# cvxgrp/cvxpygen

Measured on AMD Instinct MI355X. Metric: QP instances solved/sec (batched MPC QP, OSQP; inputs resident in HBM), higher is better.
Workload: dtype f64

## Files before the change

### cvxpygen_amd/codegen.py

```python

from __future__ import annotations

import os
import shutil
import subprocess
from typing import List, Optional, Sequence

import numpy as np

from .solve_program import GEN_EXTRA_SLOTS, LANES, RaggedProgram, execution_steps, padded_offsets_fit

CSRC = os.path.join(os.path.dirname(os.path.abspath(__file__)), 'csrc')


class ProgramTooLarge(Exception):
    """the family's solve program cannot be made LDS-resident: no specialised library for it"""


def emit_program_header(rp: RaggedProgram, name: str = 'family', plan=None, depth: int = 2, cross: int = 4,
                        pad_offsets: bool = False, group_offsets: int = 4, batch: int = 1, early: int = 4) -> str:
    out: List[str] = []
    w = out.append
    w(f'// Generated by cvxpygen_amd.codegen for problem family "{name}" -- do not edit.')
    w(f'// solve program: {rp.n_phases} phases, {rp.n_chunks} chunks, {int(rp.ctab[:, 0].sum())} steps, '
# ... 504 lines not shown
                    if int(rp.ctab[c, 3]) & 2:
                        w(f'        const double o{c} = w[r{c} & CPG_GEN_SLOT_MASK];')
                w('        cpgw::sched_fence();')
                nsteps_c = {}
                for _, c in lst:
                    nsteps_c[c] = nsteps_c.get(c, 0) + 1
                kacc = {c: (1 if (n_ < 6 or not TEAM_SPLIT_SUMS) else (2 if n_ < 12 else 4)) for c, n_ in nsteps_c.items()}
                seen, first = {}, {}
                for t, c in lst:
                    cx = f'cf[{reg_of[t]}]' if coef == 'reg' else f'c{t}'
                    j = seen.get(c, 0) % kacc[c]
                    seen[c] = seen.get(c, 0) + 1
                    nm = f'a{c}' if kacc[c] == 1 else f'a{c}_{j}'
                    if (c, j) not in first:
                        first[(c, j)] = True
                        w(f'        double {nm} = {cx} * x{t};' if coef == 'reg' else f'        double {nm} = fma({cx}, x{t}, 0.0);')
                    else:
                        w(f'        {nm} = fma({cx}, x{t}, {nm});')
                for c in chunks:
                    if kacc[c] == 2:
                        w(f'        const double a{c} = a{c}_0 + a{c}_1;')
                    elif kacc[c] == 4:
                        w(f'        const double a{c} = (a{c}_0 + a{c}_1) + (a{c}_2 + a{c}_3);')
                for c in chunks:
                    lg, kind = int(rp.ctab[c, 1]), int(rp.ctab[c, 3])
                    assert not kind & 4, 'a team executor has no deferred phases (resident_plan: intra phases instead)'
                    red = f'cpgw::seg_sum_first_lit<{lg}>(a{c}, {_mask_literals(stage_masks(rp, c, shift_of[c]))})' if kind & 1 else f'cpgw::group_sum_first<{lg}>(a{c})'
                    acc = f'o{c} + ' if kind & 2 else ''
                    w(f'        w[r{c} & CPG_GEN_SLOT_MASK] = {acc}{red};')
            if sync:
                w('        cpgw::block_sync();')
        w('    } break;')
    w('    default: {')
    if sync:
        for _ in plist:
            w('        cpgw::block_sync();')
    w('    } break;')
    w('    }')
    w('}')
    w('}  // namespace cpg')
    return '\n'.join(out) + '\n' + epilogue


def factor_fingerprint(fac) -> int:
    h = 0x811C9DC5
    ct = np.asarray(fac.ctab, dtype=np.int32).reshape(-1, 4)[:, [0, 1, 3]]
    for arr in (np.ascontiguousarray(ct), np.ascontiguousarray(fac.tlen, dtype=np.uint32)):
        for b in arr.tobytes():
            h = ((h ^ b) * 0x01000193) & 0xFFFFFFFF
    return h


FACTOR_LOOKAHEAD = int(os.environ.get('CPG_FACTOR_LOOKAHEAD', 3))


def emit_factor_program(fac, nnzL: int, N: int, prefix: str = 'GENI', lookahead: Optional[int] = None,
                        preloaded: bool = False, func: str = 'numeric_ldl_gen', zero: Optional[int] = None, body: bool = True,
                        one: Optional[int] = None, inverse_from: Optional[int] = None) -> str:
    G = f'CPG_{prefix}_FAC'
    P = FACTOR_LOOKAHEAD if lookahead is None else lookahead
    ct = np.asarray(fac.ctab, dtype=np.int64).reshape(-1, 4)
    nch = ct.shape[0]
    first = np.concatenate([[0], np.cumsum(ct[:, 0])])
    out = []
    w = out.append
    w(f'#define {G}_NCHUNKS {nch}')
    w(f'#define {G}_NSTEPS {int(first[-1])}')
    w(f'#define {G}_FINGERPRINT {factor_fingerprint(fac)}u')
    w(f'#define {G}_ZERO {nnzL + N if zero is None else int(zero)}')
    if one is not None:
        w(f'#define {G}_ONE {int(one)}')
    inv0 = nch if inverse_from is None else int(inverse_from)
    w(f'#define {G}_CHUNKS {{' + ', '.join(f'{{{int(L)}, {int(last)}, {int(lg)}}}' for L, last, _, lg in ct) + '}')
    if not body:
        return '\n'.join(out) + '\n'
    w(f'#define {G}_GENERATED 1')
    w('namespace cpg {')
    if preloaded:
        w(f'CPG_DEV void {func}(const unsigned long long *tri, const unsigned *dk, double *w, int lane) {{')
    else:
        w(f'CPG_DEV void {func}(const unsigned long long *tri, const unsigned *dk, const double *kct, const double *rinv,')
        w('                             double *w, int lane) {')
    w('    const unsigned ln = (unsigned)cpgw::opaque(lane);     // (table addresses computed here, not hoisted out of the instance loop)')

    def req_dk(c):
        if c < nch:
            w(f'    const unsigned d{c} = cpgw::gld(dk, {c * 64}u + ln);')

    def req_rest(c):
        if c < nch:
            if not preloaded and c < inv0:
                w(f'    const double kc{c} = cpgw::gld(kct, {c * 64}u + ln);')
                w(f'    const double kr{c} = cpgw::gld(rinv, (d{c} >> 16) ? (d{c} >> 16) - 1u : 0u);')
            for s_ in range(int(ct[c, 0])):
                w(f'    const unsigned long long e{int(first[c]) + s_} = cpgw::gld(tri, {(int(first[c]) + s_) * 64}u + ln);')
    for c in range(2 * P):
        req_dk(c)
    for c in range(P):
        req_rest(c)
    for c in range(nch):
        L, last, _, lg = (int(v) for v in ct[c])
        last &= 1
        w(f'    // chunk {c}: {L} step(s), groups of {1 << lg}' + (', level end' if last else ''))
        req_dk(c + 2 * P)
        req_rest(c + P)
        if preloaded and L == 0:
            if last:
                w('    cpgw::lds_order();')
            continue
        w(f'    double a{c} = 0.0;')
        for s_ in range(L):
            e = f'e{int(first[c]) + s_}'
            w(f'    a{c} = fma(w[(unsigned){e} & 0xFFFFu] * w[(unsigned)({e} >> 32)], w[((unsigned){e} >> 16)], a{c});')
        w(f'    a{c} = cpgw::group_sum_first<{lg}>(a{c});')
        w(f'    if ((d{c} & 0xFFFFu) != 0xFFFFu) {{')
        if c >= inv0 and not preloaded:
            w(f'        w[d{c} & 0xFFFFu] = -a{c};')
        elif preloaded:
            w(f'        const double v = w[d{c} & 0xFFFFu] - a{c};')
            w(f'        w[d{c} & 0xFFFFu] = (d{c} >> 16) ? 1.0 / v : v;')
        else:
            w(f'        const double v = (kc{c} - ((d{c} >> 16) ? kr{c} : 0.0)) - a{c};')
            w(f'        w[d{c} & 0xFFFFu] = (d{c} & 0xFFFFu) >= {nnzL}u ? 1.0 / v : v;')
        w('    }')
        if last:
            w('    cpgw::lds_order();')
    w('    cpgw::lds_order();')
    w('}')
# ... 89 lines not shown
    else:
        sh = stream_header(plan, out_dir, name)
        if sh is not None:
            defs.append(f'-DCPG_GENS_HEADER="{sh}"')
    return hdr, defs


GENS_MAX_STEPS = int(os.environ.get('CPG_GENS_MAX_STEPS', 1200))
GENS_LOOKAHEAD = int(os.environ.get('CPG_GENS_LOOKAHEAD', 16))


def stream_header(plan, out_dir: str, name: str = 'family') -> Optional[str]:
    from . import refactor_plan as _rp
    from .solve_program import execution_steps
    d = plan.desc
    if not matrix_parameters(d) or os.environ.get('CPG_GENS', '0') != '1':
        return None
    rpl = _rp.build_refactor_plan(d.P, d.A, plan.osqp)
    T = len(execution_steps(rpl.sol))
    if T == 0 or T > GENS_MAX_STEPS or any(int(k_) & ~1 for k_ in rpl.sol.ctab[:, 3]):
        return None
    text = emit_instance_program(rpl.sol, name, lookahead=GENS_LOOKAHEAD, prefix='GENS', func='run_program_gens', coef='mem')
    path = os.path.join(os.path.abspath(out_dir), f'cpg_stream_{name}.h')
    if not (os.path.exists(path) and open(path).read() == text):
        with open(path, 'w') as f:
            f.write(text)
    return path


GENI_MAX_REGS = int(os.environ.get('CPG_GENI_MAX_REGS', 64))
GENI_MAX_STEPS = int(os.environ.get('CPG_GENI_MAX_STEPS', 240))
LDS_BYTES = 160 * 1024


SHARED_REG_LDS_REGS = 20


def shared_register_lds_bytes(n: int, m: int, n_steps: int, n_chunks: int, n_slots: int, n_regs: int, waves: int = 8) -> int:
    tab = 2 * (256 * ((n_steps + 3) // 4) + 256 * ((n_chunks + 3) // 4))
    return 8 * (n + m) + tab + 8 * 64 * min(SHARED_REG_LDS_REGS, n_regs) + waves * 8 * (n_slots + GEN_EXTRA_SLOTS)


def instance_program_fits(rpl) -> bool:
    mg = getattr(rpl, 'merged', None)
    rp = mg.sol if mg is not None else rpl.sol
    N = rpl.n + rpl.m
    steps = execution_steps(rp)
    if len(steps) > GENI_MAX_STEPS or rp.n_slots + GEN_EXTRA_SLOTS > 0x1FFF or not np.array_equal(rp.final_pos, np.arange(N)):
        return False
    if pack_step_registers(rp, steps)[2] > GENI_MAX_REGS:
        return False
    tab = 2 * (256 * ((len(steps) + 3) // 4) + 256 * ((rp.n_chunks + 3) // 4))
    per_wave = rp.n_slots + GEN_EXTRA_SLOTS + N + (N & 1)
    fac = rpl.nnzL + N
    if mg is not None:
        fac = mg.fac_len
        if fac >= 0xFFFF:
            return False
    per_wave = max(per_wave, fac + (fac & 1))
    return tab + 8 * 8 * per_wave <= LDS_BYTES


def instance_header(plan, out_dir: str, name: str = 'family') -> Optional[str]:
    from . import refactor_plan as _rp
    d = plan.desc
    o = plan.osqp_shared or plan.osqp
    Ps, As = o.pruned(d.P, d.A)
    rpl = _rp.shared_mode_plan(Ps, As, o)
    if not instance_program_fits(rpl):
        return None
    dims = dict(N=d.n_var, M=d.m, NEQ=d.n_eq)
    mg = rpl.merged
    if mg is None:
        prog, fac = rpl.sol, emit_factor_program(rpl.fac, rpl.nnzL, rpl.n + rpl.m)
    else:
        import types
        dims['NNZX'] = mg.nnzX
        prog = mg.sol
        fac = emit_factor_program(types.SimpleNamespace(ctab=mg.f_ctab, tlen=mg.f_len), rpl.nnzL, rpl.n + rpl.m,
                                  zero=mg.fac_len - 1, one=mg.one_pos, inverse_from=mg.base.fac.n_chunks)
    return write_instance_header(prog, os.path.join(os.path.abspath(out_dir), f'cpg_instance_{name}.h'), name,
                                 row_programs=shared_row_programs(Ps, As), dims=dims, epilogue=fac, lean=True)


RESIDENT_MAX_REGS = int(os.environ.get('CPG_RESIDENT_MAX_REGS', 160))
RESIDENT_MAX_STEPS = int(os.environ.get('CPG_RESIDENT_MAX_STEPS', 320))
RESIDENT_ACC_BASE = int(os.environ.get('CPG_RESIDENT_ACC_BASE', 32))
RESIDENT_GATHER_BATCH = int(os.environ.get('CPG_RESIDENT_GATHER_BATCH', 12))
RESIDENT_ACC_PAIRS = int(os.environ.get('CPG_RESIDENT_ACC_PAIRS', 112))


def resident_compiler_flags(defs: Sequence[str]) -> List[str]:
    return []


def matrix_parameters(desc) -> bool:
    import scipy.sparse as _sps
    NP = desc.NP
    return any(_sps.csr_matrix(desc.maps[k])[:, :NP].nnz > 0 for k in ('P', 'A'))


def resident_program_fits(rpl, np_var: Optional[int] = None) -> bool:
    rp = rpl.sol
    b = rpl.base
    N = b.n + b.m
    steps = execution_steps(rp)
    if len(steps) > RESIDENT_MAX_STEPS or not np.array_equal(rp.final_pos, np.arange(N)):
        return False
    if pack_step_registers(rp, steps)[2] > RESIDENT_MAX_REGS:
        return False
    tab = 2 * (256 * ((len(steps) + 3) // 4) + 256 * ((rp.n_chunks + 3) // 4))
    np_var = b.nnzP + b.nnzA + N if np_var is None else np_var
    slice_ = max(rpl.fac_len, rpl.w_slots + N, b.nnzA + b.nnzP + max(np_var, N + max(b.n, b.m)))
    slice_ += slice_ & 1
    return 8 * slice_ <= 0xFFFF and tab + 2 * 8 * slice_ <= LDS_BYTES


def resident_four_waves(rpl, np_var: int) -> bool:
    if os.environ.get('CPG_RES_FOUR_WAVES', '0') != '1':
        return False
    b = rpl.base
    N = b.n + b.m
    slice_ = max(rpl.fac_len, rpl.w_slots + b.m, max(b.nnzA + b.nnzP, max(np_var, N + max(b.n, b.m))))
    slice_ += slice_ & 1
    return 4 * 8 * slice_ <= LDS_BYTES


def resident_header(plan, out_dir: str, name: str = 'family') -> Optional[str]:
    from . import resident_plan as _rs
    d = plan.desc
    if not matrix_parameters(d):
        return None
    rpl = _rs.build_resident_plan(d.P, d.A, plan.osqp)
# ... 686 lines not shown
```

### cvxpygen_amd/csrc/cpg_hip.cpp

```cpp
#include "../../include/cpg_hip.h"

#include <math.h>
#include <stdio.h>
#include <stdlib.h>
#include <string.h>

#include <algorithm>
#include <string>
#include <type_traits>
#include <vector>

#include "cpg_osqp_kernel.h"
#include "cpg_osqp_refactor.h"
#include "cpg_osqp_resident.h"
#include "cpg_osqp_team.h"
#include "cpg_osqp_squad.h"
#include "cpg_clarabel_kernel.h"

#include <hip/hip_runtime.h>
typedef hipStream_t rt_stream_t;
typedef hipEvent_t rt_event_t;
#define RT_CHECK(expr)                                                                         \
    do {                                                                                       \
        hipError_t e_ = (expr);                                                                \
// ... 431 lines not shown
static int launch_squad(cpg_handle_t h, const cpg::DevBatch &Bt, int blocks, size_t lds) {
    const int nsx = (h->F.n + 63) / 64, nsz = (h->F.m + 63) / 64, nv = vary_slots(h);
#define Y(a, b, v, g, wm)                                                                         \
    if (nsx == a && nsz == b && (nv <= v || (v >= a && v >= b)) && g == 1)                        \
        return launch_kernel(osqp_squad_kernel<a, b, v>, blocks, CPG_GENQ_W * 64, lds, h->stream, h->F, h->U, h->S, Bt);
    CPG_KERNELS_LDS(Y)
#undef Y
    set_error("no compiled squad kernel for this family size");
    return CPG_E_UNSUPPORTED;
}
#endif

#if defined(CPG_GENI_HEADER) && defined(CPG_GENI_NNZX)
static int shared_reg_waves(cpg_handle_t h) { return h->waves_per_block > 0 && h->waves_per_block < 8 ? h->waves_per_block : 8; }
static size_t shared_reg_lds(cpg_handle_t h, int W) {
    const size_t tab = (size_t)(((CPG_GENI_NSTEPS + 3) / 4) * 256 + ((CPG_GENI_NCHUNKS + 3) / 4) * 256) * sizeof(unsigned short);
    return (size_t)(h->F.n + h->F.m) * sizeof(double) + tab + (size_t)cpg::SharedRegExec::nlds * 64 * sizeof(double) +
           (size_t)W * (CPG_GENI_NSLOTS + CPG_GEN_EXTRA_SLOTS) * sizeof(double);
}
static bool shared_reg_usable(cpg_handle_t h) {
    return !h->refactor_mode && !h->conic && h->sreg_ok && h->sreg_rho == h->F.rho && h->sreg_sigma == h->F.sigma &&
           h->inst_per_wave == 1 && shared_reg_lds(h, shared_reg_waves(h)) <= h->lds_limit;
}
static int launch_shared_reg(cpg_handle_t h, const cpg::DevBatch &Bt, int blocks, int waves, size_t lds) {
    const int nsx = (h->F.n + 63) / 64, nsz = (h->F.m + 63) / 64, nv = vary_slots(h);
#define Y(a, b, v, g, wm)                                                                         \
    if (nsx <= a && nsz <= b && (nv <= v || (v >= a && v >= b)) && g == 1)                        \
        return launch_kernel(osqp_shared_reg_kernel<a, b, v>, blocks, waves * 64, lds, h->stream, h->F, h->U, h->S, Bt, h->SRg);
    CPG_KERNELS_LDS(Y)
#undef Y
    set_error("no compiled register-executor kernel for this family size");
    return CPG_E_UNSUPPORTED;
}
#else
static bool shared_reg_usable(cpg_handle_t) { return false; }
#endif

static cpg::DevBatch make_batch(int64_t B, const double *d_theta, const double *d_state_in, double *d_state_out, double *d_prim,
                                double *d_dual, double *d_obj, int32_t *d_iter, int32_t *d_status, double *d_pri, double *d_dua) {
    cpg::DevBatch Bt;
    Bt.scratch = nullptr; Bt.state_in = d_state_in; Bt.state_out = d_state_out;
    Bt.B = B; Bt.theta = d_theta; Bt.prim = d_prim; Bt.dual = d_dual; Bt.obj = d_obj; Bt.pri_res = d_pri;
    Bt.dua_res = d_dua; Bt.iter = d_iter; Bt.status = d_status; Bt.counter = nullptr;
    Bt.ho_list = nullptr; Bt.ho_count = nullptr; Bt.ho_state = nullptr; Bt.list = nullptr; Bt.list_count = nullptr; Bt.resume = 0;
    return Bt;
}

#ifdef CPG_GENI_HEADER
static size_t instance_kernel_lds(const cpg_solver_s *h) {
    const size_t tab = (size_t)(((CPG_GENI_NSTEPS + 3) / 4) * 256 + ((CPG_GENI_NCHUNKS + 3) / 4) * 256) * sizeof(unsigned short);
    const size_t nq = (size_t)(h->F.n + h->F.m);
    size_t per_wave = (size_t)(CPG_GENI_NSLOTS + CPG_GEN_EXTRA_SLOTS) + nq + (nq & 1);
#ifdef CPG_GENI_FAC_NSTEPS
    const size_t fac = (size_t)CPG_GENI_FAC_ZERO + 1;
#else
    const size_t fac = (size_t)h->R.nnzL + nq;
#endif
    if (per_wave < fac) per_wave = fac + (fac & 1);
    return tab + 8 * per_wave * sizeof(double);
}
static bool instance_kernel_fits(const cpg_solver_s *h) {
    return h->R.gi_ok && h->program_in_lds != 0 && h->program_in_lds != 2 && instance_kernel_lds(h) <= h->lds_limit;
}
#endif

static int launch_per_instance(cpg_handle_t h, rt_stream_t stream, const cpg::DevSettings &S, cpg::DevBatch &Bt) {
    int rc;
    auto scratch = [&](int blocks, int waves, size_t doubles) {
        const int r = ensure(h->scratch, (size_t)blocks * waves * doubles * sizeof(double));
        Bt.scratch = (double *)h->scratch.p;
        return r;
    };
#ifdef CPG_GENT_HEADER
    if (h->Rs.ok == 2 && !h->R.shared_mats && h->program_in_lds != 0 && h->program_in_lds != 2) {
        const size_t lds = ((size_t)CPG_TEAM_SLICE_OFF + (size_t)h->Rs.slice_doubles) * sizeof(double);
        if (lds <= h->lds_limit) {
            long long per_cu = (long long)(h->lds_limit / lds);
            if (per_cu * CPG_GENT_W > 16) per_cu = 16 / CPG_GENT_W;
            if (CPG_GENT_W <= 4 && per_cu * CPG_GENT_W > 4) per_cu = 4 / CPG_GENT_W;
            if (h->blocks_per_cu > 0 && per_cu > h->blocks_per_cu) per_cu = h->blocks_per_cu;
            const int blocks = std::max(1, grid_blocks(h, Bt.B, 1, per_cu));
            if ((rc = scratch(blocks, 1, h->Rs.buf_doubles))) return rc;
            return launch_kernel(osqp_team_kernel, blocks, CPG_GENT_W * 64, lds, stream, h->F, h->R, h->Rs, S, Bt);
        }
    }
#endif
#ifdef CPG_GENR_HEADER
    if (h->Rs.ok && !h->R.shared_mats && h->program_in_lds != 0 && h->program_in_lds != 2) {
#ifdef CPG_GENR_TABLES_GLOBAL
        const size_t tab = 0;
#else
        const size_t tab = (size_t)(((CPG_GENR_NSTEPS + 3) / 4) * 256 + ((CPG_GENR_NCHUNKS + 3) / 4) * 256) * sizeof(unsigned short);
#endif
        const size_t slice = (size_t)h->Rs.slice_doubles * sizeof(double);
        int NW = h->waves_per_block > 0 ? h->waves_per_block : 4;
        if (NW > 4) NW = 4;
        while (NW > 1 && tab + (size_t)NW * slice > h->lds_limit) NW--;
        const size_t lds = tab + (size_t)NW * slice;
        if (lds <= h->lds_limit) {
            const int blocks = grid_blocks(h, Bt.B, NW, 1);
            if ((rc = scratch(blocks, NW, h->Rs.buf_doubles))) return rc;
            if (slot_class(h, rc, [&](auto NSX, auto NSZ) {
                    return launch_kernel(osqp_resident_kernel<NSX, NSZ>, blocks, NW * 64, lds, stream, h->F, h->R, h->Rs, S, Bt); }))
                return rc;
        }
    }
#endif
// ... 981 lines not shown
#ifdef CPG_GENI_NNZX
    const bool merged_lib = true;
#else
    const bool merged_lib = false;
#endif
    if (!(geni_dims && (g.nnzX > 0) == merged_lib && g.sol_chunks == CPG_GENI_NCHUNKS && g.sol_nnz == CPG_GENI_NNZ && g.sol_slots == CPG_GENI_NSLOTS))
        return CPG_OK;
    const size_t nd = (size_t)r->nnzL + N, nx = (size_t)g.nnzX;
    const unsigned hsh = program_fingerprint(g.sol_ctab, g.sol_desc, g.sol_cols, g.sol_chunks, g.sol_nnz);
    static const int steps[][4] = CPG_GENI_STEPS;
    static const int chunk_shift[] = CPG_GENI_CHUNK_SHIFT;
    bool ok = hsh == CPG_GENI_FINGERPRINT;
    {
        const int nn[3] = {CPG_GENI_AROWS_N, CPG_GENI_PROWS_N, CPG_GENI_ATROWS_N};
        for (int k = 0; ok && k < 3; k++) {
            if ((int)h->rows_hdr[k].size() != 4 * nn[k]) ok = false;
            for (int c2 = 0; ok && c2 < nn[k]; c2++)
                if (h->rows_hdr[k][4 * c2] != cpg::GeniRows::len(k, c2) || h->rows_hdr[k][4 * c2 + 3] != cpg::GeniRows::off(k, c2)) ok = false;
        }
    }
    if (ok) ok = generated_tables(g.sol_ctab, g.sol_desc, g.sol_cols, g.sol_chunks, g.sol_nnz, g.sol_slots, steps, CPG_GENI_NSTEPS, gcols, grows, chunk_shift, geni_row_bytes);
    if (ok) {
        gsrc.assign((size_t)CPG_GENI_NREGS * 64, 0u);
        glcol.assign((size_t)CPG_GENI_NREGS * 64, (unsigned short)0);
        std::vector<char> taken((size_t)CPG_GENI_NREGS * 64, 0);
        for (int t = 0; ok && t < CPG_GENI_NSTEPS; t++) {
            const int e = steps[t][0], cnt = steps[t][1], reg = steps[t][2], sh = steps[t][3];
            if (reg < 0 || reg >= CPG_GENI_NREGS) { ok = false; break; }
            for (int l = 0; l < cnt; l++) {
                int kind = g.sol_kind[e + l], idx = g.sol_idx[e + l];
                if (kind == 4) {
                    if (idx < 0 || (size_t)idx >= nx) { ok = false; break; }
                    kind = 3; idx += (int)N;
                }
                if (kind < 0 || kind > 3 || idx < 0 || idx >= (1 << 28)) { ok = false; break; }
                const size_t at = (size_t)reg * 64 + (size_t)(l + sh);
                if (taken[at]) { ok = false; break; }
                taken[at] = 1;
                gsrc[at] = ((unsigned)kind << 28) | (unsigned)idx;
                if (kind == 2) {
                    if (idx >= r->nnzL || r->Lcol[idx] < 0 || r->Lcol[idx] > 0xFFFF) { ok = false; break; }
                    glcol[at] = (unsigned short)r->Lcol[idx];
                }
            }
        }
    }
#ifdef CPG_GENI_FAC_NSTEPS
    if (ok) {
        static const int fch[][3] = CPG_GENI_FAC_CHUNKS;
        const size_t fac_end = nx ? nd + nx + 2 : nd + 1;
        const size_t one = nd + nx;
        unsigned hsh2 = 0x811C9DC5u;
        auto mix = [&](unsigned v) { for (int k = 0; k < 4; k++) { hsh2 = (hsh2 ^ ((v >> (8 * k)) & 0xFFu)) * 0x01000193u; } };
        ok = g.fac_chunks == CPG_GENI_FAC_NCHUNKS && fac_end - 1 == (size_t)CPG_GENI_FAC_ZERO && fac_end <= 0xFFFFu;
#ifdef CPG_GENI_FAC_ONE
        ok = ok && one == (size_t)CPG_GENI_FAC_ONE;
#endif
        for (int c = 0; ok && c < g.fac_chunks; c++) { mix((unsigned)g.fac_ctab[4 * c]); mix((unsigned)g.fac_ctab[4 * c + 1]); mix((unsigned)g.fac_ctab[4 * c + 3]); }
        for (size_t e = 0; ok && e < (size_t)g.fac_chunks * 64; e++) mix(g.fac_len[e]);
        ok = ok && hsh2 == CPG_GENI_FAC_FINGERPRINT;
        if (ok) {
            const unsigned long long Z = (unsigned long long)(fac_end - 1);
            gtri.assign((size_t)CPG_GENI_FAC_NSTEPS * 64, Z | (Z << 16) | (Z << 32));
            gdk.assign((size_t)g.fac_chunks * 64, 0xFFFFu);
            gkc.assign((size_t)g.fac_chunks * 64, 0.0);
            size_t step = 0;
            for (int c = 0; ok && c < g.fac_chunks; c++) {
                const int L = g.fac_ctab[4 * c];
                size_t base = (size_t)g.fac_ctab[4 * c + 2];
                if (L != fch[c][0]) { ok = false; break; }
                for (int s = 0; ok && s < L; s++, step++) {
                    int cnt = 0;
                    for (int l = 0; l < 64; l++) {
                        const unsigned ln = g.fac_len[(size_t)c * 64 + l];
                        if ((int)(ln & 0xFFFFu) <= s) continue;
                        const size_t e = base + (size_t)l;
                        if (l != cnt || e >= (size_t)g.fac_triples) { ok = false; break; }
                        cnt++;
                        if ((int)(ln >> 16) > s) {
                            const unsigned a = g.fac_a[e], b = g.fac_b[e], k = nx ? g.fac_k[e] : (unsigned)r->nnzL + g.fac_k[e];
                            if (a >= (unsigned)r->nnzL || !(b < (unsigned)r->nnzL || (nx && b >= nd && b <= one)) ||
                                k < (unsigned)r->nnzL || k >= nd) { ok = false; break; }
                            gtri[step * 64 + (size_t)l] = (unsigned long long)a | ((unsigned long long)b << 16) | ((unsigned long long)k << 32);
                        }
                    }
                    base += (size_t)cnt;
                }
                for (int l = 0; ok && l < 64; l++) {
                    const unsigned t0 = g.fac_task[(size_t)c * 64 + l];
                    if (t0 == 0xFFFFFFFFu) continue;
                    const unsigned t = nx ? (t0 & 0x7FFFFFFFu) : t0;
                    if (t >= nd + nx) { ok = false; break; }
                    const int kr = t < nd ? fkrow[t] : -1;
                    gdk[(size_t)c * 64 + l] = t | ((unsigned)(kr + 1) << 16);
                    gkc[(size_t)c * 64 + l] = t < nd ? fkc[t] : 0.0;
                }
            }
            if (ok && step != (size_t)CPG_GENI_FAC_NSTEPS) ok = false;
        }
        if (ok) {
            if ((rc = upload<unsigned long long>(h, own, gtri.data(), gtri.size(), &R.gf_tri))) return rc;
            if ((rc = upload<unsigned>(h, own, gdk.data(), gdk.size(), &R.gf_dk))) return rc;
            if ((rc = upload<double>(h, own, gkc.data(), gkc.size(), &R.gf_kc))) return rc;
        }
    }
#else
    ok = ok && !nx;
#endif
    if (ok) {
        if ((rc = upload<unsigned short>(h, own, glcol.data(), glcol.size(), &R.gi_lcol))) return rc;
        if ((rc = upload<unsigned short>(h, own, gcols.data(), gcols.size(), &R.gi_cols))) return rc;
        if ((rc = upload<unsigned short>(h, own, grows.data(), grows.size(), &R.gi_rows))) return rc;
        if ((rc = upload<unsigned>(h, own, gsrc.data(), gsrc.size(), &R.gi_src))) return rc;
    }
    if ((rc = rt_sync(h))) return rc;
    R.gi_ok = ok ? 1 : 0;
    return CPG_OK;
// ... 1067 lines not shown
```

### cvxpygen_amd/csrc/cpg_osqp_refactor.h

```cpp
#pragma once

#include "cpg_osqp_kernel.h"

#ifdef CPG_GENI_HEADER
#include CPG_GENI_HEADER
#endif
#ifdef CPG_GENS_HEADER
#include CPG_GENS_HEADER
#define CPG_GENS_ACTIVE(geni, shared, crlds) (!(geni) && !(shared) && !(crlds))
#else
#define CPG_GENS_ACTIVE(geni, shared, crlds) false
#endif

namespace cpg {

#ifdef CPG_GENI_HEADER
struct GeniRows {
    static constexpr int len(int which, int s) {
        constexpr int a[][2] = CPG_GENI_AROWS; constexpr int p[][2] = CPG_GENI_PROWS; constexpr int t[][2] = CPG_GENI_ATROWS;
        return which == 0 ? (s < CPG_GENI_AROWS_N ? a[s < CPG_GENI_AROWS_N ? s : 0][0] : 0)
             : which == 1 ? (s < CPG_GENI_PROWS_N ? p[s < CPG_GENI_PROWS_N ? s : 0][0] : 0)
                          : (s < CPG_GENI_ATROWS_N ? t[s < CPG_GENI_ATROWS_N ? s : 0][0] : 0);
    }
    static constexpr int off(int which, int s) {
        constexpr int a[][2] = CPG_GENI_AROWS; constexpr int p[][2] = CPG_GENI_PROWS; constexpr int t[][2] = CPG_GENI_ATROWS;
        return which == 0 ? a[s < CPG_GENI_AROWS_N ? s : 0][1] : which == 1 ? p[s < CPG_GENI_PROWS_N ? s : 0][1]
                                                                            : t[s < CPG_GENI_ATROWS_N ? s : 0][1];
    }
};
#define CPG_GENI_ROWS(P, which, s, w, lane) natural_chunk_lit(P, GeniRows::len(which, s), GeniRows::off(which, s), w, lane)
#endif

struct DevRefactor {
    int nnzP, nnzA, nnzL, n_eq, np_var, scaling_iters;
    const int *Ap, *Ai, *Arp, *Aent, *Acol, *Pp, *Pi, *Prp, *Pent, *Pcol;
    const int *Lcol, *ksrc_kind, *ksrc_idx;
    const int *fac_ctab;
    const unsigned *fac_task, *fac_len, *fac_a, *fac_b, *fac_k;
    int fac_chunks;
    const int *sol_kind, *sol_idx;
    const unsigned short *sol_fpos;
    int sol_nnz, sol_slots;
    const unsigned *sol_stab;
    const unsigned *sol_cr;
    int sol_pairs;
    const double *P_base, *A_base, *q_base, *u_base;
    const double *q_setup;
    double d_base;
    DevCsr map_P, map_A, map_q, map_u, map_d;
    long long buf_doubles;
    int shared_mats;
    const double *Ps, *As, *Ars, *Ds, *Dinvs, *Es, *Einvs;
    double cs;
    int gi_ok;
    const unsigned short *gi_cols, *gi_rows;
    const unsigned *gi_src;
    const unsigned short *gi_lcol;
    const unsigned long long *gf_tri;
// ... 336 lines not shown
        double c[CPG_GENI_NREGS];
#pragma unroll
        for (int t = 0; t < CPG_GENI_NREGS; t++) c[t] = t < nreg ? cf[t < nreg ? t : 0] : lcf[(unsigned)(t - nreg) * 64u + (unsigned)lane];
        run_program_inst(c, lc, lr, w, lane);
    }
};
#endif
#endif

CPG_DEV double uniform_double(double v) {
    int w2[2];
    __builtin_memcpy(w2, &v, 8);
    w2[0] = cpgw::read_first_lane(w2[0]); w2[1] = cpgw::read_first_lane(w2[1]);
    __builtin_memcpy(&v, w2, 8);
    return v;
}

template <int NSX, int NSZ, bool GENI = false, bool SHARED = GENI, bool CRLDS = false>
CPG_DEV void osqp_refactor_body(const DevFamily &F0, const DevRefactor &R, const DevSettings &S,
                                const DevBatch &Bt, double *lds, int wave_global) {
    const int lane = cpgw::lane_id();
#if defined(CPG_GENI_HEADER) && defined(CPG_GENI_N)
    const unsigned n = GENI ? (unsigned)CPG_GENI_N : (unsigned)F0.n, m = GENI ? (unsigned)CPG_GENI_M : (unsigned)F0.m, N = n + m;
    const unsigned n_eq = GENI ? (unsigned)CPG_GENI_NEQ : (unsigned)R.n_eq;
#else
    const unsigned n = (unsigned)F0.n, m = (unsigned)F0.m, N = n + m, n_eq = (unsigned)R.n_eq;
#endif
    const unsigned *cr_tab = R.sol_cr;
    if (CRLDS) {
        unsigned *lc = (unsigned *)lds;
        const unsigned ncr = (unsigned)R.sol_nnz;
        for (unsigned t = cpgw::thread_in_block(); t < ncr; t += cpgw::block_threads()) lc[t] = cpgw::gld(R.sol_cr, t);
        cpgw::block_sync();
        cr_tab = lc;
        lds += (ncr + 1u) / 2u;
    }
#ifdef CPG_GENI_HEADER
    const int ldw = GENI ? CPG_GENI_NSLOTS + CPG_GEN_EXTRA_SLOTS : (CPG_GENS_ACTIVE(GENI, SHARED, CRLDS) ? R.sol_slots + CPG_GEN_EXTRA_SLOTS : R.sol_slots);
    constexpr unsigned gi_ncols = ((CPG_GENI_NSTEPS + 3u) / 4u) * 256u, gi_nrows = ((CPG_GENI_NCHUNKS + 3u) / 4u) * 256u;
    const unsigned short *gi_lc = nullptr, *gi_lr = nullptr;
    if (GENI) {
        unsigned short *lc = (unsigned short *)lds, *lr = lc + gi_ncols;
        for (unsigned t = cpgw::thread_in_block(); t < gi_ncols; t += cpgw::block_threads()) lc[t] = cpgw::gld(R.gi_cols, t);
        for (unsigned t = cpgw::thread_in_block(); t < gi_nrows; t += cpgw::block_threads()) lr[t] = cpgw::gld(R.gi_rows, t);
        cpgw::block_sync();
        gi_lc = lc; gi_lr = lr;
        lds += (gi_ncols + gi_nrows) / 4u;
    }
#else
    const int ldw = CPG_GENS_ACTIVE(GENI, SHARED, CRLDS) ? R.sol_slots + CPG_GEN_EXTRA_SLOTS : R.sol_slots;
#endif
    size_t per_wave = (size_t)ldw + (GENI ? (size_t)(N + (N & 1u)) : 0u);
#ifdef CPG_GENI_FAC_NSTEPS
    const size_t fac_doubles = (size_t)CPG_GENI_FAC_ZERO + 1u;
#else
    const size_t fac_doubles = (size_t)R.nnzL + N;
#endif
    if (GENI && per_wave < fac_doubles) per_wave = fac_doubles + (fac_doubles & 1u);
    double *w = lds + (size_t)cpgw::wave_in_block() * per_wave;
    double *qs = w + ldw, *us = qs + n;
    constexpr bool shared = SHARED || GENI;
#ifdef CPG_GENS_HEADER
    constexpr bool GENS = !shared && !CRLDS;
#else
    constexpr bool GENS = false;
#endif
    InstBuf B = carve(Bt.scratch + (size_t)wave_global * (size_t)R.buf_doubles, F0, R);
    const double rho_fr = CPG_RHO_MIN, ri_fr = 1.0 / rho_fr;
    const size_t state_len = (size_t)n + 2u * (size_t)m + 1u;
    unsigned short fpx[NSX], fpz[NSZ];
#pragma unroll
    for (int s = 0; s < NSX; s++) { const unsigned i = (unsigned)lane + 64u * (unsigned)s; fpx[s] = i < n ? cpgw::gld(R.sol_fpos, i) : 0; }
#pragma unroll
    for (int s = 0; s < NSZ; s++) { const unsigned i = (unsigned)lane + 64u * (unsigned)s; fpz[s] = i < m ? cpgw::gld(R.sol_fpos, n + i) : 0; }

    const unsigned n_work = Bt.list_count ? cpgw::sld(Bt.list_count, 0u) : 0u;
    if (shared) {
        B.P = const_cast<double *>(R.Ps); B.A = const_cast<double *>(R.As); B.Ar = const_cast<double *>(R.Ars);
        B.D = const_cast<double *>(R.Ds); B.Dinv = const_cast<double *>(R.Dinvs);
        B.E = const_cast<double *>(R.Es); B.Einv = const_cast<double *>(R.Einvs);
    }

    for (;;) {
        unsigned ig = 0;
        if (lane == 0) ig = cpgw::atomic_next(Bt.counter);
        ig = (unsigned)cpgw::read_first_lane((int)ig);
        long long b = (long long)ig;
        if (Bt.list) {
            if (ig >= n_work) break;
            b = (long long)cpgw::read_first_lane(cpgw::gld(Bt.list, ig));
        } else if (b >= Bt.B) break;
        const double *theta = Bt.theta + (size_t)b * R.np_var;
        const double *state_in = (Bt.state_in && (S.warm_starting || Bt.resume)) ? Bt.state_in + (size_t)b * state_len : nullptr;
        double rho = Bt.state_in ? cpgw::gld(Bt.state_in + (size_t)b * state_len, n + 2u * m) : F0.rho;
        rho = cpgw::dmin2(cpgw::dmax2(rho, CPG_RHO_MIN), CPG_RHO_MAX);
        if (GENI) rho = uniform_double(rho);
        double rho_stg = F0.rho;
        double rho_eq = 1e3 * rho, rho_in = rho, ri_eq = 1.0 / rho_eq, ri_in = 1.0 / rho_in;

        const bool probe = GENI && __builtin_expect(S.debug_stage == 20, 0);
        unsigned long long ts[8];
        int n_ts = 0;
#define CPG_INST_PROBE() do { if (GENI && probe && n_ts < 8) ts[n_ts++] = cpgw::clock100(); } while (0)
        CPG_INST_PROBE();
#ifdef CPG_GENI_HEADER
        double cf[CPG_GENI_NREGS];
        signed char fct[NSZ];
#pragma unroll
        for (int s = 0; s < NSZ; s++) fct[s] = 0;
        const bool fam_start = GENI && R.fam_cf != nullptr && rho == R.fam_rho && F0.sigma == R.fam_sigma;
        if (GENI && fam_start) {
            const unsigned ln = (unsigned)cpgw::opaque(lane);
#pragma unroll
            for (int s = 0; s < NSZ; s++) { const unsigned i = ln + 64u * (unsigned)s; fct[s] = i < m ? cpgw::gld(R.fam_ct, i) : (signed char)0; }
        }
#endif
        if (!shared) {
            for (unsigned k = (unsigned)lane; k < (unsigned)R.nnzA; k += 64u) cpgw::gst(B.A, k, csr_row(R.map_A, k, theta, cpgw::gld(R.A_base, k)));
            for (unsigned k = (unsigned)lane; k < (unsigned)R.nnzP; k += 64u) cpgw::gst(B.P, k, csr_row(R.map_P, k, theta, cpgw::gld(R.P_base, k)));
        }
        double qv[GENI ? NSX : 1], uv[GENI ? NSZ : 1];
        if (GENI) {
            const unsigned ln = (unsigned)cpgw::opaque(lane);
#pragma unroll
            for (int s = 0; s < NSX; s++) {
                const unsigned i = ln + 64u * (unsigned)s;
                qv[GENI ? s : 0] = 0.0;
                if ((unsigned)lane + 64u * (unsigned)s < n) { qv[GENI ? s : 0] = csr_row(R.map_q, i, theta, cpgw::gld(R.q_base, i)); cpgw::gst(B.q, i, qv[GENI ? s : 0]); }
            }
#pragma unroll
            for (int s = 0; s < NSZ; s++) {
                const unsigned i = ln + 64u * (unsigned)s;
                uv[GENI ? s : 0] = 0.0;
                if ((unsigned)lane + 64u * (unsigned)s < m) { uv[GENI ? s : 0] = csr_row(R.map_u, i, theta, cpgw::gld(R.u_base, i)); cpgw::gst(B.u, i, uv[GENI ? s : 0]); }
            }
        } else {
            for (unsigned i = (unsigned)lane; i < n; i += 64u) cpgw::gst(B.q, i, csr_row(R.map_q, i, theta, cpgw::gld(R.q_base, i)));
            for (unsigned i = (unsigned)lane; i < m; i += 64u) cpgw::gst(B.u, i, csr_row(R.map_u, i, theta, cpgw::gld(R.u_base, i)));
        }
        const double dconst = csr_row(R.map_d, 0, theta, R.d_base);
        if (!GENI) cpgw::mem_order();
        double cs = shared ? R.cs : 1.0;
        if (!shared) {
#ifdef CPG_REFACTOR_ROW_COPY
            refresh_row_copy(R, B, lane);
#endif

            for (unsigned i = (unsigned)lane; i < N; i += 64u) w[i] = 1.0;
            cpgw::lds_order();
#pragma nounroll
            for (int it = 0; it < R.scaling_iters; it++) {
                double dn[NSX], en[NSZ];
#pragma unroll
                for (int s = 0; s < NSX; s++) {
                    const unsigned j = (unsigned)lane + 64u * (unsigned)s;
                    double acc = 0.0;
// ... 57 lines not shown
#ifdef CPG_REFACTOR_ROW_COPY
            refresh_row_copy(R, B, lane);
#endif
        }
        if (__builtin_expect(S.debug_stage == 1, 0)) { if (lane == 0) { Bt.status[b] = 11; Bt.iter[b] = 0; } continue; }
        signed char ct[NSZ];
        const int lane_rc = GENI ? cpgw::opaque(lane) : lane;
#pragma unroll
        for (int s = 0; s < NSZ; s++) {
            const unsigned i = (unsigned)lane_rc + 64u * (unsigned)s;
            const unsigned ic = (unsigned)lane + 64u * (unsigned)s;
            ct[s] = 0;
            if (ic < m) {
                double uu = GENI ? uv[GENI ? s : 0] : cpgw::gld((const double *)B.u, i);
                if (!shared) {
                    const double ei = w[n + i];
                    uu = ei * uu;
                    cpgw::gst(B.E, i, ei); cpgw::gst(B.Einv, i, 1.0 / ei); cpgw::gst(B.u, i, uu);
                }
                ct[s] = ic < n_eq ? 1 : (uu > CPG_INFTY * CPG_MIN_SCALING ? -1 : 0);
                cpgw::gst(B.rinv, i, ct[s] == 1 ? ri_eq : (ct[s] == 0 ? ri_in : ri_fr));
            }
        }
        if (!GENI) { cpgw::lds_order(); cpgw::mem_order(); }
        double rvv[NSZ], riv[NSZ];
        auto set_steps = [&]() __attribute__((always_inline)) {
#pragma unroll
            for (int s = 0; s < NSZ; s++) {
                rvv[s] = ct[s] == 1 ? rho_eq : (ct[s] == 0 ? rho_in : rho_fr);
                riv[s] = ct[s] == 1 ? ri_eq : (ct[s] == 0 ? ri_in : ri_fr);
            }
        };
        if (GENI) set_steps();

        auto factor_generic = [&]() __attribute__((always_inline)) {
            if (shared) {
                cpgw::mem_order();
                numeric_ldl_m<false>(R, B.Lx, B.Dginv, (const double *)B.rinv, lane);
                substitution_values<true>(R, B, lane);
            } else {
                numeric_ldl(R, B, F0.sigma, lane);
                substitution_values<false, GENS>(R, B, lane);
            }
        };
#ifdef CPG_GENI_HEADER
        auto factor_in_lds = [&]() __attribute__((always_inline)) {
            cpgw::mem_order();
#ifdef CPG_GENI_FAC_NSTEPS
            if (lane == 0) w[CPG_GENI_FAC_ZERO] = 0.0;
#ifdef CPG_GENI_FAC_ONE
            if (lane == 0) w[CPG_GENI_FAC_ONE] = 1.0;
#endif
            cpgw::lds_order();
            numeric_ldl_gen(R.gf_tri, R.gf_dk, R.gf_kc, (const double *)B.rinv, w, lane);
#else
            numeric_ldl_m<true>(R, w, w + R.nnzL, (const double *)B.rinv, lane);
#endif
            load_instance_coefficients(R, w, w + R.nnzL, cf, lane);
            cpgw::lds_order();
            for (unsigned t = (unsigned)lane; t < (unsigned)ldw; t += 64u) w[t] = 0.0;
            for (unsigned i = (unsigned)lane; i < n; i += 64u) qs[i] = cpgw::gld((const double *)B.q, i);
            for (unsigned i = (unsigned)lane; i < m; i += 64u) us[i] = cpgw::gld((const double *)B.u, i);
            cpgw::lds_order();
        };
        if (__builtin_expect(S.debug_stage == 2, 0)) { if (lane == 0) { Bt.status[b] = 11; Bt.iter[b] = 0; } continue; }
        CPG_INST_PROBE();
        if (GENI) {
            bool other = false;
#pragma unroll
            for (int s = 0; s < NSZ; s++) other = other || ((unsigned)lane + 64u * (unsigned)s < m && ct[s] != fct[s]);
            if (fam_start && cpgw::ballot(other) == 0ull) {
                const unsigned ln = (unsigned)cpgw::opaque(lane);
#pragma unroll
                for (int t = 0; t < CPG_GENI_NREGS; t++) cf[t] = cpgw::gld(R.fam_cf, (unsigned)t * 64u + ln);
                for (unsigned t = (unsigned)lane; t < (unsigned)ldw; t += 64u) w[t] = 0.0;
#pragma unroll
                for (int s = 0; s < NSX; s++) { const unsigned i = (unsigned)lane + 64u * (unsigned)s; if (i < n) qs[i] = qv[GENI ? s : 0]; }
#pragma unroll
                for (int s = 0; s < NSZ; s++) { const unsigned i = (unsigned)lane + 64u * (unsigned)s; if (i < m) us[i] = uv[GENI ? s : 0]; }
                cpgw::lds_order();
            } else factor_in_lds();
        }
        else
#endif
        factor_generic();
        if (__builtin_expect(S.debug_stage == 3, 0)) { if (lane == 0) { Bt.status[b] = 11; Bt.iter[b] = 0; } continue; }
#ifdef CPG_GENI_HEADER
        if (GENI && __builtin_expect(S.debug_stage == 21, 0)) {
            const int rsel = (int)(b % (long long)CPG_GENI_NREGS);
            double v = 0.0;
#pragma unroll
            for (int t = 0; t < CPG_GENI_NREGS; t++) v = t == rsel ? cf[t] : v;
            if (F0.n_prim >= 64) Bt.prim[(size_t)b * F0.n_prim + (unsigned)lane] = v;
            if (lane == 0) { Bt.status[b] = 11; Bt.iter[b] = 0; }
            continue;
        }
#endif
        CPG_INST_PROBE();

#ifdef CPG_GENS_HEADER
        if (GENS) {
            if (lane == 0) w[CPG_GENS_NSLOTS + CPG_GEN_DUMMY_SLOTS] = 0.0;
            cpgw::lds_order();
        }
#endif
        DevFamily F = F0;
        F.D = B.D; F.Dinv = B.Dinv; F.E = B.E; F.Einv = B.Einv; F.c = cs; F.cinv = 1.0 / cs;
        StreamProg ST;
        ST.stab = R.sol_stab; ST.cr = cr_tab; ST.vals = B.sv;
        ST.n_pairs = R.sol_pairs; ST.dummy = (unsigned)R.sol_nnz / 2u - 1u;
        typedef InstCtx<NSX, NSZ, GENI> CtxT;
        double qr[NSX], ur[NSZ];
// ... 278 lines not shown
```

Before: 6.199 million.

## Generate level-scheduled LDL factor program with batched gathers and per-kind reciprocal

Adds a by-level emitter for the generated numeric LDL factorisation. Chunks are grouped into dependency levels. All gathers of a level are issued before one sched fence, and one LDS ordering barrier replaces the per-chunk ones. Global table loads are requested a bounded number of levels ahead, and chunks are classified so that pivot chunks always take a reciprocal and plain chunks skip the select. Idle lanes now write to two extra dummy LDS doubles instead of an out-of-range slot, which enlarges the per-wave LDS footprint. Debug timing probes and asm region markers are also added.

New measurement: 6.299 million, median of 6. 1.02x the previous value.

```diff
diff --git a/cvxpygen_amd/codegen.py b/cvxpygen_amd/codegen.py
--- a/cvxpygen_amd/codegen.py
+++ b/cvxpygen_amd/codegen.py
@@ -580,11 +580,118 @@
 
 
 FACTOR_LOOKAHEAD = int(os.environ.get('CPG_FACTOR_LOOKAHEAD', 3))
+FACTOR_BY_LEVEL = os.environ.get('CPG_FACTOR_BY_LEVEL', '1') != '0'
+FACTOR_LOOKAHEAD_CHUNKS = int(os.environ.get('CPG_FACTOR_LOOKAHEAD_CHUNKS', 3))
+FACTOR_DUMMY_DOUBLES = 2
+
+
+def factor_levels(ctab) -> List[List[int]]:
+    ct = np.asarray(ctab, dtype=np.int64).reshape(-1, 4)
+    levels, cur = [], []
+    for c in range(ct.shape[0]):
+        cur.append(c)
+        if int(ct[c, 1]) & 1:
+            levels.append(cur)
+            cur = []
+    if cur:
+        levels.append(cur)
+    return levels
+
+
+def factor_chunk_kinds(fac, nnzL: int, N: int, inverse_from: Optional[int] = None) -> List[str]:
+    ct = np.asarray(fac.ctab, dtype=np.int64).reshape(-1, 4)
+    nch = ct.shape[0]
+    task = np.asarray(fac.task, dtype=np.int64).reshape(nch, -1)
+    inv0 = nch if inverse_from is None else int(inverse_from)
+    kinds = []
+    for c in range(nch):
+        t = task[c][task[c] != 0xFFFFFFFF] & 0x7FFFFFFF
+        piv = (t >= nnzL) & (t < nnzL + N)
+        kinds.append('inverse' if c >= inv0 else ('pivot' if len(t) and piv.all() else ('mixed' if piv.any() else 'plain')))
+    return kinds
+
+
+def _emit_factor_levels(fac, ct, first, nnzL: int, N: int, G: str, P: int, func: str, inv0: int) -> str:
+    nch = ct.shape[0]
+    levels = factor_levels(ct)
+    kinds = factor_chunk_kinds(fac, nnzL, N, inv0)
+    out = []
+    w = out.append
+    w(f'#define {G}_GENERATED 1')
+    w(f'#define {G}_BY_LEVEL 1')
+    w(f'#define {G}_NLEVELS {len(levels)}')
+    w(f'#define {G}_NLEVELS_WITH_STEPS {sum(1 for lv in levels if any(int(ct[c, 0]) for c in lv))}')
+    w(f'// chunks: {kinds.count("pivot")} pivot (reciprocal, no select), {kinds.count("mixed")} mixed (reciprocal and select), '
+      f'{kinds.count("plain")} plain, {kinds.count("inverse")} inverse; {sum(1 for c in range(nch) if int(ct[c, 0]) == 0)} without a step')
+    w('namespace cpg {')
+    w(f'CPG_DEV void {func}(const unsigned long long *tri, const unsigned *dk, const double *kct, const double *rinv,')
+    w('                             double *w, int lane) {')
+    w('    const unsigned ln = (unsigned)cpgw::opaque(lane);     // (table addresses computed here, not hoisted out of the instance loop)')
+
+    def req_dk(lv):
+        for c in (levels[lv] if lv < len(levels) else ()):
+            w(f'    const unsigned d{c} = cpgw::gld(dk, {c * 64}u + ln);')
+
+    def req_rest(lv):
+        for c in (levels[lv] if lv < len(levels) else ()):
+            if c < inv0:
+                w(f'    const double kc{c} = cpgw::gld(kct, {c * 64}u + ln);')
+                w(f'    const double kr{c} = cpgw::gld(rinv, (d{c} >> 16) ? (d{c} >> 16) - 1u : 0u);')
+            for s_ in range(int(ct[c, 0])):
+                w(f'    const unsigned long long e{int(first[c]) + s_} = cpgw::gld(tri, {(int(first[c]) + s_) * 64}u + ln);')
+    def request_points(ahead, budget):
+        rp = []
+        for L in range(len(levels)):
+            j = max(L - ahead, rp[-1] if rp else 0, 0)
+            while j < L and sum(len(levels[l]) for l in range(j, L + 1)) > budget:
+                j += 1
+            rp.append(j)
+        return rp
+    at_dk, at_rest = request_points(2 * P, 2 * FACTOR_LOOKAHEAD_CHUNKS), request_points(P, FACTOR_LOOKAHEAD_CHUNKS)
+    at_dk = [min(a, b) for a, b in zip(at_dk, at_rest)]
+    for lv, chunks in enumerate(levels):
+        w(f'    // level {lv}: chunk(s) ' + ', '.join(f'{c} ({int(ct[c, 0])} step(s), groups of {1 << int(ct[c, 3])}, {kinds[c]})' for c in chunks))
+        for L in range(lv, len(levels)):
+            if at_dk[L] == lv:
+                req_dk(L)
+        for L in range(lv, len(levels)):
+            if at_rest[L] == lv:
+                req_rest(L)
+        steps = [int(first[c]) + s_ for c in chunks for s_ in range(int(ct[c, 0]))]
+        for e in steps:
+            w(f'    const double ga{e} = w[(unsigned)e{e} & 0xFFFFu], gk{e} = w[(unsigned)(e{e} >> 32)], gb{e} = w[((unsigned)e{e} >> 16)];')
+        if steps:
+            w('    cpgw::sched_fence();')
+        for c in chunks:
+            L, lg = int(ct[c, 0]), int(ct[c, 3])
+            if L:
+                w(f'    double a{c} = 0.0;')
+                for s_ in range(L):
+                    e = int(first[c]) + s_
+                    w(f'    a{c} = fma(ga{e} * gk{e}, gb{e}, a{c});')
+                w(f'    a{c} = cpgw::group_sum_first<{lg}>(a{c});')
+            if kinds[c] == 'inverse':
+                w(f'    const double v{c} = {"-a%d" % c if L else "-0.0"};')
+                continue
+            base = f'(kc{c} - ((d{c} >> 16) ? kr{c} : 0.0))'
+            w(f'    const double u{c} = {base + (" - a%d" % c if L else "")};')
+            if kinds[c] == 'plain':
+                w(f'    const double v{c} = u{c};')
+            elif kinds[c] == 'pivot':
+                w(f'    const double v{c} = 1.0 / u{c};')
+            else:
+                w(f'    const double v{c} = (d{c} & 0xFFFFu) >= {nnzL}u ? 1.0 / u{c} : u{c};')
+        for c in chunks:
+            w(f'    w[d{c} & 0xFFFFu] = v{c};')
+        w('    cpgw::lds_order();')
+    w('}')
+    w('}  // namespace cpg')
+    return '\n'.join(out) + '\n'
 
 
 def emit_factor_program(fac, nnzL: int, N: int, prefix: str = 'GENI', lookahead: Optional[int] = None,
                         preloaded: bool = False, func: str = 'numeric_ldl_gen', zero: Optional[int] = None, body: bool = True,
-                        one: Optional[int] = None, inverse_from: Optional[int] = None) -> str:
+                        one: Optional[int] = None, inverse_from: Optional[int] = None, by_level: bool = False) -> str:
     G = f'CPG_{prefix}_FAC'
     P = FACTOR_LOOKAHEAD if lookahead is None else lookahead
     ct = np.asarray(fac.ctab, dtype=np.int64).reshape(-1, 4)
@@ -602,6 +709,9 @@
     w(f'#define {G}_CHUNKS {{' + ', '.join(f'{{{int(L)}, {int(last)}, {int(lg)}}}' for L, last, _, lg in ct) + '}')
     if not body:
         return '\n'.join(out) + '\n'
+    if by_level:
+        assert not preloaded
+        return '\n'.join(out) + '\n' + _emit_factor_levels(fac, ct, first, nnzL, N, G, P, func, inv0)
     w(f'#define {G}_GENERATED 1')
     w('namespace cpg {')
     if preloaded:
@@ -797,11 +907,13 @@
         return False
     tab = 2 * (256 * ((len(steps) + 3) // 4) + 256 * ((rp.n_chunks + 3) // 4))
     per_wave = rp.n_slots + GEN_EXTRA_SLOTS + N + (N & 1)
-    fac = rpl.nnzL + N
+    fac = rpl.nnzL + N + 1
     if mg is not None:
         fac = mg.fac_len
-        if fac >= 0xFFFF:
-            return False
+    if FACTOR_BY_LEVEL:
+        fac += FACTOR_DUMMY_DOUBLES
+    if mg is not None and fac >= 0xFFFF:
+        return False
     per_wave = max(per_wave, fac + (fac & 1))
     return tab + 8 * 8 * per_wave <= LDS_BYTES
 
@@ -817,13 +929,13 @@
     dims = dict(N=d.n_var, M=d.m, NEQ=d.n_eq)
     mg = rpl.merged
     if mg is None:
-        prog, fac = rpl.sol, emit_factor_program(rpl.fac, rpl.nnzL, rpl.n + rpl.m)
+        prog, fac = rpl.sol, emit_factor_program(rpl.fac, rpl.nnzL, rpl.n + rpl.m, by_level=FACTOR_BY_LEVEL)
     else:
         import types
         dims['NNZX'] = mg.nnzX
         prog = mg.sol
-        fac = emit_factor_program(types.SimpleNamespace(ctab=mg.f_ctab, tlen=mg.f_len), rpl.nnzL, rpl.n + rpl.m,
-                                  zero=mg.fac_len - 1, one=mg.one_pos, inverse_from=mg.base.fac.n_chunks)
+        fac = emit_factor_program(types.SimpleNamespace(ctab=mg.f_ctab, tlen=mg.f_len, task=mg.f_task), rpl.nnzL, rpl.n + rpl.m,
+                                  zero=mg.fac_len - 1, one=mg.one_pos, inverse_from=mg.base.fac.n_chunks, by_level=FACTOR_BY_LEVEL)
     return write_instance_header(prog, os.path.join(os.path.abspath(out_dir), f'cpg_instance_{name}.h'), name,
                                  row_programs=shared_row_programs(Ps, As), dims=dims, epilogue=fac, lean=True)
 
diff --git a/cvxpygen_amd/csrc/cpg_hip.cpp b/cvxpygen_amd/csrc/cpg_hip.cpp
--- a/cvxpygen_amd/csrc/cpg_hip.cpp
+++ b/cvxpygen_amd/csrc/cpg_hip.cpp
@@ -507,7 +507,7 @@
     const size_t nq = (size_t)(h->F.n + h->F.m);
     size_t per_wave = (size_t)(CPG_GENI_NSLOTS + CPG_GEN_EXTRA_SLOTS) + nq + (nq & 1);
 #ifdef CPG_GENI_FAC_NSTEPS
-    const size_t fac = (size_t)CPG_GENI_FAC_ZERO + 1;
+    const size_t fac = (size_t)CPG_GENI_FAC_ZERO + 1 + CPG_GENI_FAC_DUMMY_DOUBLES;
 #else
     const size_t fac = (size_t)h->R.nnzL + nq;
 #endif
@@ -1595,7 +1595,8 @@
         const size_t one = nd + nx;
         unsigned hsh2 = 0x811C9DC5u;
         auto mix = [&](unsigned v) { for (int k = 0; k < 4; k++) { hsh2 = (hsh2 ^ ((v >> (8 * k)) & 0xFFu)) * 0x01000193u; } };
-        ok = g.fac_chunks == CPG_GENI_FAC_NCHUNKS && fac_end - 1 == (size_t)CPG_GENI_FAC_ZERO && fac_end <= 0xFFFFu;
+        const unsigned idle_dst = CPG_GENI_FAC_DUMMY_DOUBLES ? (unsigned)fac_end : 0xFFFFu;
+        ok = g.fac_chunks == CPG_GENI_FAC_NCHUNKS && fac_end - 1 == (size_t)CPG_GENI_FAC_ZERO && fac_end + CPG_GENI_FAC_DUMMY_DOUBLES <= 0xFFFFu;
 #ifdef CPG_GENI_FAC_ONE
         ok = ok && one == (size_t)CPG_GENI_FAC_ONE;
 #endif
@@ -1605,7 +1606,7 @@
         if (ok) {
             const unsigned long long Z = (unsigned long long)(fac_end - 1);
             gtri.assign((size_t)CPG_GENI_FAC_NSTEPS * 64, Z | (Z << 16) | (Z << 32));
-            gdk.assign((size_t)g.fac_chunks * 64, 0xFFFFu);
+            gdk.assign((size_t)g.fac_chunks * 64, idle_dst);
             gkc.assign((size_t)g.fac_chunks * 64, 0.0);
             size_t step = 0;
             for (int c = 0; ok && c < g.fac_chunks; c++) {
diff --git a/cvxpygen_amd/csrc/cpg_osqp_refactor.h b/cvxpygen_amd/csrc/cpg_osqp_refactor.h
--- a/cvxpygen_amd/csrc/cpg_osqp_refactor.h
+++ b/cvxpygen_amd/csrc/cpg_osqp_refactor.h
@@ -4,6 +4,16 @@
 
 #ifdef CPG_GENI_HEADER
 #include CPG_GENI_HEADER
+#endif
+#ifdef CPG_GENI_FAC_BY_LEVEL
+#define CPG_GENI_FAC_DUMMY_DOUBLES 2u
+#else
+#define CPG_GENI_FAC_DUMMY_DOUBLES 0u
+#endif
+#if defined(__HIP_DEVICE_COMPILE__)
+#define CPG_REGION_MARK(s) asm volatile("; cpg-region " s)
+#else
+#define CPG_REGION_MARK(s) ((void)0)
 #endif
 #ifdef CPG_GENS_HEADER
 #include CPG_GENS_HEADER
@@ -446,7 +456,7 @@
 #endif
     size_t per_wave = (size_t)ldw + (GENI ? (size_t)(N + (N & 1u)) : 0u);
 #ifdef CPG_GENI_FAC_NSTEPS
-    const size_t fac_doubles = (size_t)CPG_GENI_FAC_ZERO + 1u;
+    const size_t fac_doubles = (size_t)CPG_GENI_FAC_ZERO + 1u + CPG_GENI_FAC_DUMMY_DOUBLES;
 #else
     const size_t fac_doubles = (size_t)R.nnzL + N;
 #endif
@@ -492,10 +502,11 @@
         double rho_stg = F0.rho;
         double rho_eq = 1e3 * rho, rho_in = rho, ri_eq = 1.0 / rho_eq, ri_in = 1.0 / rho_in;
 
-        const bool probe = GENI && __builtin_expect(S.debug_stage == 20, 0);
+        const bool probe = GENI && __builtin_expect(S.debug_stage == 20 || S.debug_stage == 24, 0);
         unsigned long long ts[8];
         int n_ts = 0;
 #define CPG_INST_PROBE() do { if (GENI && probe && n_ts < 8) ts[n_ts++] = cpgw::clock100(); } while (0)
+#define CPG_INST_PROBE_SPLIT() do { if (GENI && probe && S.debug_stage == 24 && n_ts < 8) ts[n_ts++] = cpgw::clock100(); } while (0)
         CPG_INST_PROBE();
 #ifdef CPG_GENI_HEADER
         double cf[CPG_GENI_NREGS];
@@ -659,12 +670,18 @@
             if (lane == 0) w[CPG_GENI_FAC_ONE] = 1.0;
 #endif
             cpgw::lds_order();
+            CPG_REGION_MARK("factor begin");
             numeric_ldl_gen(R.gf_tri, R.gf_dk, R.gf_kc, (const double *)B.rinv, w, lane);
+            CPG_REGION_MARK("factor end");
 #else
             numeric_ldl_m<true>(R, w, w + R.nnzL, (const double *)B.rinv, lane);
 #endif
+            CPG_INST_PROBE_SPLIT();
+            CPG_REGION_MARK("coefficients begin");
             load_instance_coefficients(R, w, w + R.nnzL, cf, lane);
+            CPG_REGION_MARK("coefficients end");
             cpgw::lds_order();
+            CPG_INST_PROBE_SPLIT();
             for (unsigned t = (unsigned)lane; t < (unsigned)ldw; t += 64u) w[t] = 0.0;
             for (unsigned i = (unsigned)lane; i < n; i += 64u) qs[i] = cpgw::gld((const double *)B.q, i);
             for (unsigned i = (unsigned)lane; i < m; i += 64u) us[i] = cpgw::gld((const double *)B.u, i);
```
